# adamjorr/kbbq-py

Hardware: NVIDIA B200
Metric: bases/sec recalibrated (table build + apply) (higher is better)
Workload: dtype u8 in/out, u32->int64 counts, f64 model

## Files before the change

include/kbbq_b200.h:

```cpp
#ifndef KBBQ_B200_H
#define KBBQ_B200_H

#include <stddef.h>
#include <stdint.h>

#ifdef __cplusplus
extern "C" {
#endif

#define KBBQ_NQ 43
#define KBBQ_NDINUC 16

#define KBBQ_OK 0
#define KBBQ_E_ARG (-1)
#define KBBQ_E_CUDA (-2)
#define KBBQ_E_WORKSPACE (-3)
#define KBBQ_E_DATA (-4)
#define KBBQ_E_IO (-5)
#define KBBQ_E_FORMAT (-6)
#define KBBQ_E_RAGGED (-7)
#define KBBQ_E_NAME_FIELD (-8)
#define KBBQ_E_NAME_RG (-9)
#define KBBQ_E_NAME_MISMATCH (-10)
#define KBBQ_E_PEER (-11)
// ... 24 lines not shown
                   int64_t *rg_total_dev, int64_t *meanq_dev, void *stream);

int kbbq_delta_q(const int64_t *prior_q_dev, const int64_t *numerrs_dev,
                 const int64_t *numtotal_dev, int64_t n, int64_t *delta_dev, void *stream);

int kbbq_posterior_q_real(const double *prior_q_dev, const int64_t *numerrs_dev,
                          const int64_t *numtotal_dev, int64_t n, int64_t *posterior_dev, void *stream);

int kbbq_bam_workspace_bytes(int64_t N, int L, int R, size_t *bytes);
int kbbq_build_bam(const uint8_t *seq_dev, const uint8_t *qual_dev, const uint8_t *err_dev,
                   const uint8_t *skip_dev, const uint16_t *rg_dev, const uint8_t *flags_dev,
                   const uint16_t *aln_start_dev, const uint16_t *aln_end_dev, int64_t N, int L, int R,
                   int minscore, int64_t *pos_errs_dev, int64_t *pos_total_dev, int64_t *din_errs_dev,
                   int64_t *din_total_dev, void *workspace_dev, size_t workspace_bytes, int *status_dev,
                   void *stream);
int kbbq_apply_bam(const uint8_t *seq_dev, const uint8_t *qual_dev, const uint16_t *rg_dev,
                   const uint8_t *flags_dev, int64_t N, int L, int R, int minscore,
                   const int64_t *meanq_dev, const int64_t *rgdq_dev, const int64_t *qdq_dev,
                   const int64_t *posdq_dev, const int64_t *dindq_dev, int nq, int ndin1,
                   uint8_t *out_qual_dev, void *workspace_dev, size_t workspace_bytes, int *status_dev,
                   void *stream);

int kbbq_calibration_counts(const uint8_t *qual_dev, const uint8_t *err_dev, const uint8_t *seq_dev,
                            const uint8_t *corr_dev, const uint8_t *skip_dev, int64_t n,
                            int64_t *total_dev, int64_t *errs_dev, void *stream);

int kbbq_get_delta_qs(const int64_t *meanq_dev, const int64_t *rg_errs_dev,
                      const int64_t *rg_total_dev, const int64_t *q_errs_dev,
                      const int64_t *q_total_dev, const int64_t *pos_errs_dev,
                      const int64_t *pos_total_dev, const int64_t *din_errs_dev,
                      const int64_t *din_total_dev, int R, int nq, int ncyc, int ndin,
                      int64_t *rgdq_dev, int64_t *qdq_dev, int64_t *posdq_dev, int64_t *dindq_dev,
                      void *stream);

#define KBBQ_APPLY_BASES_CHECKED 0x10
int kbbq_apply(const uint8_t *seq_dev, const uint8_t *qual_dev, const uint16_t *rg_dev,
               const uint8_t *second_dev, int64_t N, int L, int R, int minscore,
               const int64_t *meanq_dev, const int64_t *rgdq_dev, const int64_t *qdq_dev,
               const int64_t *posdq_dev, const int64_t *dindq_dev, int nq, int ndin1,
               uint8_t *out_qual_dev, void *workspace_dev, size_t workspace_bytes, int *status_dev,
               int path, void *stream);

int64_t kbbq_segment_rows_bound(int64_t N, int R);
int64_t kbbq_segment_table_elems(int R);
int kbbq_segmented_supported(int L, int R, int minscore);
int kbbq_segment_plan(const uint16_t *rg_dev, const uint8_t *second_dev, int64_t N, int R, uint32_t *seg_dev,
                      uint32_t *dest_dev, int *status_dev, void *stream);
int kbbq_segment_rows(const uint8_t *src_dev, const uint32_t *dest_dev, int64_t N, int L, uint8_t *dst_segmented_dev,
                      void *stream);
int kbbq_segment_pad(const uint32_t *seg_dev, int R, int L, uint8_t *seq_dev, uint8_t *qual_dev, uint8_t *corr_dev,
                     void *stream);
int kbbq_unsegment_rows(const uint8_t *src_segmented_dev, const uint32_t *dest_dev, int64_t N, int L,
                        int64_t rows_bound, uint8_t *dst_dev, void *stream);
int kbbq_build_segmented(const uint8_t *seq_dev, const uint8_t *qual_dev, const uint8_t *corr_dev,
                         const uint32_t *seg_dev, int64_t rows_bound, int L, int R, int minscore,
                         int64_t *pos_errs_dev, int64_t *pos_total_dev, int64_t *din_errs_dev,
                         int64_t *din_total_dev, void *workspace_dev, size_t workspace_bytes, int *status_dev,
                         void *stream);
int kbbq_apply_segmented(const uint8_t *seq_dev, const uint8_t *qual_dev, const uint32_t *seg_dev, int64_t rows_bound,
                         int L, int R, int minscore, const int64_t *meanq_dev, const int64_t *rgdq_dev,
                         const int64_t *qdq_dev, const int64_t *posdq_dev, const int64_t *dindq_dev, int nq,
                         int ndin1, uint8_t *out_qual_dev, void *workspace_dev, size_t workspace_bytes,
                         int *status_dev, void *stream);
int kbbq_apply_segmented_flags(const uint8_t *seq_dev, const uint8_t *qual_dev, const uint32_t *seg_dev,
                               int64_t rows_bound, int L, int R, int minscore, const int64_t *meanq_dev,
                               const int64_t *rgdq_dev, const int64_t *qdq_dev, const int64_t *posdq_dev,
// ... 113 lines not shown
```

kbbq-py_b200/csrc/host_api.cu:

```cuda
#include <algorithm>
#include <atomic>
#include <chrono>
#include <condition_variable>
#include <memory>
#include <mutex>
#include <sched.h>
#include <stdlib.h>
#include <string.h>
#include <sys/mman.h>
#include <sys/stat.h>
#include <fcntl.h>
#include <thread>
#include <unistd.h>
#include <vector>

#include "common.cuh"

using namespace kbbq;

namespace {

#define KBBQ_TRY(x) do { int rc_ = (x); if (rc_) return rc_; } while (0)

constexpr int MAX_DEVICES = 16;
// ... 309 lines not shown
        uint8_t *sseq = keep ? r->seq : u.sseq, *squal = keep ? r->qual : u.squal;
        KBBQ_TRY(kbbq_segment_plan(p.d_rg, p.d_sec, n, R, seg, dest, S->d_status, S->s_comp));
        KBBQ_TRY(kbbq_segment_rows(p.d_seq, dest, n, L, sseq, S->s_comp));
        KBBQ_TRY(kbbq_segment_rows(p.d_qual, dest, n, L, squal, S->s_comp));
        KBBQ_TRY(kbbq_segment_rows(u.corr, dest, n, L, u.scorr, S->s_comp));
        KBBQ_TRY(kbbq_segment_pad(seg, R, L, sseq, squal, u.scorr, S->s_comp));
        KBBQ_TRY(kbbq_build_segmented(sseq, squal, u.scorr, seg, S->rowsC, L, R, S->minscore, pe, pt, de, dt, S->d_ws,
                                      S->ws_bytes, S->d_status, S->s_comp));
    } else {
        KBBQ_TRY(kbbq_build(p.d_seq, p.d_qual, u.corr, p.d_rg, p.d_sec, n, L, R, S->minscore, pe, pt, de, dt, S->d_ws, S->ws_bytes,
                            S->d_status, 0, S->s_comp));
    }
    KBBQ_CUDA(cudaEventRecord(u.consumed, S->s_comp));
    return KBBQ_OK;
}

int build_chunk_async(kbbq_session *S, const uint8_t *seq, const uint8_t *qual, const uint8_t *corr, const uint16_t *rg,
                      const uint8_t *second, int64_t n, bool keep) {
    if (n < 0 || n > S->C) return KBBQ_E_ARG;
    if (n == 0) return KBBQ_OK;
    if (!seq || !qual || !corr) return KBBQ_E_ARG;
    const int64_t k = S->built;
    if (keep && k >= (int64_t)S->res.size()) return KBBQ_E_ARG;
    S->built++;
    KBBQ_TRY(build_chunk_upload(S, k, seq, qual, rg, second, n, keep));
    return build_chunk_finish(S, k, seq, corr, rg != nullptr, second != nullptr, n, keep);
}

int model_async(kbbq_session *S) {
    const int L = S->L, R = S->R;
    const size_t npos = (size_t)R * NQ * 2 * L, ndin = (size_t)R * NQ * 16;
    int64_t *pe = S->summed ? S->d_sum : S->d_tab, *pt = pe + npos, *de = pt + npos, *dt = de + ndin;
    const ModelPtrs &mp = S->mp;
    KBBQ_TRY(kbbq_marginals(pe, pt, L, R, mp.q_errs, mp.q_total, mp.rg_errs, mp.rg_total, mp.meanq, S->s_comp));
    KBBQ_TRY(kbbq_get_delta_qs(mp.meanq, mp.rg_errs, mp.rg_total, mp.q_errs, mp.q_total, pe, pt, de, dt, R, NQ, 2 * L, 16,
                               mp.rgdq, mp.qdq, mp.posdq, mp.dindq, S->s_comp));
    return KBBQ_OK;
}

int apply_and_download(kbbq_session *S, const uint8_t *d_seq, const uint8_t *d_qual, const uint16_t *d_rg,
                       const uint8_t *d_sec, const uint32_t *seg, const uint32_t *dest, int64_t n, uint8_t *out_host) {
    const int L = S->L, R = S->R;
    OutSlot &o = S->down[S->applied++ & 1];
    const ModelPtrs &mp = S->mp;
    KBBQ_CUDA(cudaStreamWaitEvent(S->s_comp, o.drained, 0));
    if (S->segmode) {
        KBBQ_TRY(kbbq_apply_segmented(d_seq, d_qual, seg, S->rowsC, L, R, S->minscore, mp.meanq, mp.rgdq, mp.qdq, mp.posdq,
                                      mp.dindq, NQ, 17, o.out_seg, S->d_ws, S->ws_bytes, S->d_status, S->s_comp));
        KBBQ_TRY(kbbq_unsegment_rows(o.out_seg, dest, n, L, S->rowsC, o.out, S->s_comp));
    } else {
        KBBQ_TRY(kbbq_apply(d_seq, d_qual, d_rg, d_sec, n, L, R, S->minscore, mp.meanq, mp.rgdq, mp.qdq, mp.posdq, mp.dindq,
                            NQ, 17, o.out, S->d_ws, S->ws_bytes, S->d_status, 0, S->s_comp));
    }
    KBBQ_CUDA(cudaEventRecord(o.applied, S->s_comp));
    KBBQ_CUDA(cudaStreamWaitEvent(S->s_down, o.applied, 0));
    KBBQ_CUDA(cudaMemcpyAsync(out_host, o.out, (size_t)n * L, cudaMemcpyDeviceToHost, S->s_down));
    S->d2h_bytes += n * L;
    KBBQ_CUDA(cudaEventRecord(o.drained, S->s_down));
    return KBBQ_OK;
}

int apply_resident_async(kbbq_session *S, int64_t k, uint8_t *out_host) {
    if (k < 0 || k >= (int64_t)S->res.size() || !out_host) return KBBQ_E_ARG;
    const Resident &r = S->res[(size_t)k];
    if (r.n == 0) return KBBQ_OK;
    return apply_and_download(S, r.seq, r.qual, r.rg, r.sec, r.seg, r.dest, r.n, out_host);
}

int apply_chunk_async(kbbq_session *S, const uint8_t *seq, const uint8_t *qual, const uint16_t *rg, const uint8_t *second,
// ... 924 lines not shown
```

kbbq-py_b200/csrc/kbbq_b200.cu:

```cuda
#include <algorithm>
#include <mutex>
#include <stdlib.h>
#include <string.h>
#include <vector>

#include "apply.cuh"
#include "bam.cuh"
#include "build.cuh"
#include "calib.cuh"
#include "common.cuh"
#include "expand.cuh"
#include "model.cuh"
#include "prepare.cuh"
#include "segment.cuh"
#include "synth.cuh"

namespace kbbq {

std::atomic<long long> g_launches{0};
char g_last_cuda_error[256] = "";

static std::mutex g_const_mu;
static bool g_const_done[64];

// ... 105 lines not shown
};

template <class Generic>
static int plan_and_prepare(int narr, bool aligned, int64_t N, int L, int R, int minscore, const uint16_t *rg,
                            const uint8_t *second, void *workspace, size_t workspace_bytes, int *status, int path,
                            const unsigned int *seg_rows, cudaStream_t st, const Generic &generic, SmemPlan *p) {
    const bool segmode = seg_rows != nullptr;
    int device, max_smem;
    int rc = current_device_info(&device, &p->sms, &max_smem);
    if (rc) return rc;
    p->smem = path != 2 && aligned && plan_kernel(L, R, minscore, narr, max_smem, &p->g, &p->tc, &p->sl, segmode) &&
              (uint64_t)((N + p->g.G - 1) / p->g.G) < 0xFFFFFFFFull;
    if (!p->smem) {
        if (path == 1 || segmode) return KBBQ_E_ARG;
        return generic(0, N, p->sms * 8);
    }
    p->w = carve_workspace(workspace, N, L, R);
    if (!workspace || workspace_bytes < p->w.bytes) return KBBQ_E_WORKSPACE;
    p->N = N;
    if (segmode) {
        seg_prepare_kernel<<<1, 256, 0, st>>>(seg_rows, 2 * R, p->g.G, (unsigned long long)N, p->w.seg, p->w.uni, status);
        KBBQ_LAUNCHED();
        return KBBQ_OK;
    }
    const int64_t tail = (R == 1 && N > p->g.G) ? N % p->g.G : 0;
    if (tail) {
        p->N = N - tail;
        rc = generic(p->N, tail, 1);
        if (rc) return rc;
    }
    return run_prepare(rg, second, p->N, p->g.G, R, p->w, status, p->sms, p->sl.ngs, p->g.gbytes, p->sl.slot, st);
}

template <class Launch>
static int launch_bam_chunks(long long N, int L, const Launch &launch) {
    const unsigned int wmax = (unsigned int)((3 + L + 3) >> 2);
    const long long per = std::max<long long>(1, (long long)(0x7FFFFFFFu / wmax) / 256 * 256);
    for (long long r0 = 0; r0 < N; r0 += per) {
        const long long n = std::min<long long>(per, N - r0);
        launch((unsigned)((n * wmax + BAM_WARPS * 32 - 1) / (BAM_WARPS * 32)), r0, wmax);
        KBBQ_LAUNCHED();
    }
    return KBBQ_OK;
}

}

using namespace kbbq;

extern "C" {

int kbbq_abi_version(void) { return 1; }

const char *kbbq_strerror(int code) {
    switch (code) {
    case KBBQ_OK: return "ok";
    case KBBQ_E_ARG: return "bad argument";
    case KBBQ_E_CUDA: return "CUDA runtime error";
    case KBBQ_E_WORKSPACE: return "workspace too small";
    case KBBQ_E_DATA: return "input data error (see status flags)";
    case KBBQ_E_IO: return "FASTQ file could not be opened, read or written";
    case KBBQ_E_FORMAT: return "malformed FASTQ (4-line records expected)";
    case KBBQ_E_RAGGED: return "reads of unequal length";
    case KBBQ_E_NAME_FIELD: return "read name has no read-group field";
    case KBBQ_E_NAME_RG: return "read-group field does not start with RG";
    case KBBQ_E_NAME_MISMATCH: return "corrected read name does not start with the read name";
// ... 247 lines not shown
    const int grid = sms * 3;
    const long long chunk = (long long)grid * CAL_THREADS * CAL_MAX_ITERS * 32;
    auto kern = err ? (skip ? calibration_kernel<true, true> : calibration_kernel<true, false>)
                    : (skip ? calibration_kernel<false, true> : calibration_kernel<false, false>);
    KBBQ_CUDA(cudaFuncSetAttribute(kern, cudaFuncAttributeMaxDynamicSharedMemorySize, CAL_SMEM));
    for (long long o = 0; o < n; o += chunk) {
        CalibArgs c = a;
        c.qual += o; if (err) c.err += o; else { c.seq += o; c.corr += o; } if (skip) c.skip += o;
        c.n = std::min<long long>(chunk, n - o);
        kern<<<grid, CAL_THREADS, CAL_SMEM, st>>>(c);
        KBBQ_LAUNCHED();
    }
    return KBBQ_OK;
}

int kbbq_get_delta_qs(const int64_t *meanq, const int64_t *rg_errs, const int64_t *rg_total,
                      const int64_t *q_errs, const int64_t *q_total, const int64_t *pos_errs,
                      const int64_t *pos_total, const int64_t *din_errs, const int64_t *din_total, int R,
                      int nq, int ncyc, int ndin, int64_t *rgdq, int64_t *qdq, int64_t *posdq,
                      int64_t *dindq, void *stream) {
    if (R < 1 || nq < 1 || ncyc < 0 || ndin < 0) return KBBQ_E_ARG;
    if (!meanq || !rg_errs || !rg_total || !q_errs || !q_total || !rgdq || !qdq) return KBBQ_E_ARG;
    if ((ncyc && (!pos_errs || !pos_total || !posdq)) || !dindq || (ndin && (!din_errs || !din_total)))
        return KBBQ_E_ARG;
    int rc = upload_constants();
    if (rc) return rc;
    cudaStream_t st = (cudaStream_t)stream;
    DeltaArgs a = {(const long long *)meanq, (const long long *)rg_errs, (const long long *)rg_total,
                   (const long long *)q_errs, (const long long *)q_total, (const long long *)pos_errs,
                   (const long long *)pos_total, (const long long *)din_errs, (const long long *)din_total,
                   R, nq, ncyc, ndin, (long long *)rgdq, (long long *)qdq, (long long *)posdq, (long long *)dindq};
    delta_levels12_kernel<<<R, 64, 0, st>>>(a);
    KBBQ_LAUNCHED();
    const long long cells = (long long)R * nq * (ncyc + ndin + 1);
    delta_level3_kernel<<<(unsigned)((cells + 127) / 128), 128, 0, st>>>(a);
    KBBQ_LAUNCHED();
    return KBBQ_OK;
}

static int apply_impl(const uint8_t *seq, const uint8_t *qual, const uint16_t *rg, const uint8_t *second, int64_t N,
                      int L, int R, int minscore, const int64_t *meanq, const int64_t *rgdq, const int64_t *qdq,
                      const int64_t *posdq, const int64_t *dindq, int nq, int ndin1, uint8_t *out_qual,
                      void *workspace, size_t workspace_bytes, int *status, int path, void *stream,
                      const unsigned int *seg_rows) {
    const bool segmode = seg_rows != nullptr;
    const bool validate = !(path & KBBQ_APPLY_BASES_CHECKED);
    path &= ~KBBQ_APPLY_BASES_CHECKED;
    if (N < 0 || L < 1 || R < 1 || R > 65535 || minscore < 0 || minscore >= NQ) return KBBQ_E_ARG;
    if (nq < 1 || nq > NQ || ndin1 < 16 || ndin1 > 64) return KBBQ_E_ARG;
    if (!meanq || !rgdq || !qdq || !posdq || !dindq || !status) return KBBQ_E_ARG;
    if (N == 0) return KBBQ_OK;
    if (!seq || !qual || !out_qual) return KBBQ_E_ARG;
    cudaStream_t st = (cudaStream_t)stream;
    Workspace w = carve_workspace(workspace, N, L, R);
    if (!workspace || workspace_bytes < w.bytes) return KBBQ_E_WORKSPACE;

    const long long fold_cells = (long long)R * NQ * (2 * L + 16);
    fold_kernel<<<(unsigned)((fold_cells + 255) / 256), 256, 0, st>>>(
        (const long long *)meanq, (const long long *)rgdq, (const long long *)qdq, (const long long *)posdq,
        (const long long *)dindq, R, nq, 2 * L, ndin1, w.fold_cyc, w.fold_din);
    KBBQ_LAUNCHED();

    auto generic = [&](int64_t r0, int64_t n, int grid) {
        ApplyGenericArgs a = {seq + r0 * L, qual + r0 * L, rg ? rg + r0 : nullptr, second ? second + r0 : nullptr,
                              out_qual + r0 * L, n, L, R, minscore, nq, w.fold_cyc, w.fold_din, status, validate};
        apply_generic_kernel<<<grid, 256, 0, st>>>(a);
        KBBQ_LAUNCHED();
        return KBBQ_OK;
// ... 146 lines not shown
```

kbbq-py_b200/csrc/model.cuh:

```cuda
#pragma once
#include "common.cuh"

namespace kbbq {

__constant__ double c_lnp[NQ];
__constant__ double c_ln1mp[NQ];
__constant__ double c_prior[NQ];
__constant__ double c_p[NQ];
__constant__ double c_bound_hi[NQ];
__constant__ double c_bound_lo[NQ];

struct dd { double hi, lo; };
__device__ __forceinline__ dd two_sum(double a, double b) {
    double s = __dadd_rn(a, b), bb = __dsub_rn(s, a);
    double e = __dadd_rn(__dsub_rn(a, __dsub_rn(s, bb)), __dsub_rn(b, bb));
    return {s, e};
}
__device__ __forceinline__ dd two_prod(double a, double b) {
    double p = __dmul_rn(a, b);
    return {p, __fma_rn(a, b, -p)};
}
__device__ __forceinline__ dd dd_add(dd a, dd b) {
    dd s = two_sum(a.hi, b.hi);
    double lo = __dadd_rn(s.lo, __dadd_rn(a.lo, b.lo));
    return two_sum(s.hi, lo);
}
__device__ __forceinline__ dd dd_div_d(dd a, double b) {
    double q1 = __ddiv_rn(a.hi, b);
    dd p = two_prod(q1, b);
    double r = __dadd_rn(__dsub_rn(__dsub_rn(a.hi, p.hi), p.lo), a.lo);
    double q2 = __ddiv_rn(r, b);
    return two_sum(q1, q2);
}
__device__ __forceinline__ bool dd_le(dd a, double bh, double bl) {
    return a.hi < bh || (a.hi == bh && a.lo <= bl);
}

__global__ void marginals_q_kernel(const long long *pos_errs, const long long *pos_total, int L2,
                                   long long *q_errs, long long *q_total) {
    const int q = blockIdx.x, rg = blockIdx.y;
    const size_t base = ((size_t)rg * NQ + q) * L2;
    long long e = 0, t = 0;
    for (int c = threadIdx.x; c < L2; c += blockDim.x) { e += pos_errs[base + c]; t += pos_total[base + c]; }
    __shared__ long long se[32], st[32];
    for (int o = 16; o; o >>= 1) { e += __shfl_down_sync(0xFFFFFFFFu, e, o); t += __shfl_down_sync(0xFFFFFFFFu, t, o); }
    if ((threadIdx.x & 31) == 0) { se[threadIdx.x >> 5] = e; st[threadIdx.x >> 5] = t; }
    __syncthreads();
    if (threadIdx.x == 0) {
        e = 0; t = 0;
        for (int w = 0; w < (blockDim.x + 31) / 32; ++w) { e += se[w]; t += st[w]; }
        q_errs[rg * NQ + q] = e;
        q_total[rg * NQ + q] = t;
    }
}

__global__ void marginals_rg_kernel(const long long *q_errs, const long long *q_total, int R,
                                    long long *rg_errs, long long *rg_total, long long *meanq) {
    const int rg = blockIdx.x;
    __shared__ long long s_e[NQ], s_t[NQ];
    if (threadIdx.x < NQ) {
        s_e[threadIdx.x] = q_errs[rg * NQ + threadIdx.x];
        s_t[threadIdx.x] = q_total[rg * NQ + threadIdx.x];
    }
    __syncthreads();
    if (threadIdx.x != 0) return;
    long long e = 0, t = 0;
    dd acc = {0.0, 0.0};
    for (int q = 0; q < NQ; ++q) {
        const long long tq = s_t[q];
        e += s_e[q];
        t += tq;
        if (tq) acc = dd_add(acc, two_prod((double)tq, c_p[q]));
    }
    rg_errs[rg] = e;
    rg_total[rg] = t;
    long long mq = 0;
    if (t > 0) {
        if (acc.hi == 0.0) mq = NQ - 1;
        else {
            const dd p = dd_div_d(acc, (double)t);
            for (int m = 1; m < NQ; ++m) mq += dd_le(p, c_bound_hi[m], c_bound_lo[m]) ? 1 : 0;
        }
    }
    meanq[rg] = mq;
}

__device__ __forceinline__ dd round_to_x87(dd s) {
    if (s.lo == 0.0 || isinf(s.hi) || isnan(s.hi)) return s;
    int e;
    frexp(s.hi, &e);
    int eh = e - 1;
    if (fabs(s.hi) == ldexp(1.0, eh) && ((s.hi > 0.0) != (s.lo > 0.0))) eh -= 1;
    const int qe = eh - 63;
    const double lo_r = ldexp(rint(ldexp(s.lo, -qe)), qe);
    const double h = __dadd_rn(s.hi, lo_r);
    return {h, __dadd_rn(__dsub_rn(s.hi, h), lo_r)};
}

template <typename PRIOR>
__device__ __forceinline__ int posterior_q_cell(PRIOR prior, long long errs, long long tot) {
    const double k = (double)(errs + 1), mm = (double)((tot + 2) - (errs + 1));
    int best = 0;
    double bh = 0.0, bl = 0.0;
    bool have = false;
    for (int c = 0; c < NQ; ++c) {
        int d = (int)((PRIOR)c - prior);
        d = d < 0 ? -d : d;
        const double pr = d < NQ ? c_prior[d] : -KBBQ_INF;
        const double a = __dmul_rn(k, c_lnp[c]);
        const double b = (mm == 0.0) ? 0.0 : __dmul_rn(mm, c_ln1mp[c]);
        const double ll = __dadd_rn(a, b);
        double h, l;
        if (isinf(pr) || isinf(ll)) { h = -KBBQ_INF; l = 0.0; }
        else { dd s = round_to_x87(two_sum(pr, ll)); h = s.hi; l = s.lo; }
        if (!have || h > bh || (h == bh && l > bl)) { best = c; bh = h; bl = l; have = true; }
    }
    return best;
}
__device__ __forceinline__ int delta_q_cell(int prior, long long errs, long long tot) {
    return posterior_q_cell<int>(prior, errs, tot) - prior;
}

__global__ void delta_q_kernel(const long long *prior, const long long *errs, const long long *tot,
                               long long n, long long *out) {
    long long i = (long long)blockIdx.x * blockDim.x + threadIdx.x;
    if (i < n) out[i] = delta_q_cell((int)prior[i], errs[i], tot[i]);
}

__global__ void posterior_q_real_kernel(const double *prior, const long long *errs, const long long *tot,
                                        long long n, long long *out) {
    long long i = (long long)blockIdx.x * blockDim.x + threadIdx.x;
    if (i < n) out[i] = posterior_q_cell<double>(prior[i], errs[i], tot[i]);
}

struct DeltaArgs {
    const long long *meanq, *rg_errs, *rg_total, *q_errs, *q_total, *pos_errs, *pos_total, *din_errs, *din_total;
    int R, nq, ncyc, ndin;
    long long *rgdq, *qdq, *posdq, *dindq;
};

__global__ void delta_levels12_kernel(DeltaArgs a) {
    const int rg = blockIdx.x;
    __shared__ int s_prior1;
    if (threadIdx.x == 0) {
        const int mq = (int)a.meanq[rg];
        const int d = delta_q_cell(mq, a.rg_errs[rg], a.rg_total[rg]);
        a.rgdq[rg] = d;
        s_prior1 = mq + d;
    }
    __syncthreads();
    for (int q = threadIdx.x; q < a.nq; q += blockDim.x)
        a.qdq[rg * a.nq + q] = delta_q_cell(s_prior1, a.q_errs[rg * a.nq + q], a.q_total[rg * a.nq + q]);
}

__global__ void delta_level3_kernel(DeltaArgs a) {
    const long long ncell_pos = (long long)a.R * a.nq * a.ncyc;
    const long long ncell_din = (long long)a.R * a.nq * (a.ndin + 1);
    long long i = (long long)blockIdx.x * blockDim.x + threadIdx.x;
    if (i < ncell_pos) {
        const long long gq = i / a.ncyc;
        const int rg = (int)(gq / a.nq);
        const int prior2 = (int)(a.meanq[rg] + a.rgdq[rg] + a.qdq[gq]);
        a.posdq[i] = delta_q_cell(prior2, a.pos_errs[i], a.pos_total[i]);
    } else if (i < ncell_pos + ncell_din) {
        i -= ncell_pos;
        const long long gq = i / (a.ndin + 1);
        const int d = (int)(i - gq * (a.ndin + 1));
        if (d == a.ndin) { a.dindq[i] = 0; return; }
        const int rg = (int)(gq / a.nq);
        const int prior2 = (int)(a.meanq[rg] + a.rgdq[rg] + a.qdq[gq]);
        a.dindq[i] = delta_q_cell(prior2, a.din_errs[gq * a.ndin + d], a.din_total[gq * a.ndin + d]);
    }
}

__global__ void fold_kernel(const long long *meanq, const long long *rgdq, const long long *qdq,
                            const long long *posdq, const long long *dindq, int R, int nq, int L2,
                            int ndin1, short *fold_cyc, short *fold_din) {
    const long long ncyc = (long long)R * NQ * L2, ndin = (long long)R * NQ * 16;
    long long i = (long long)blockIdx.x * blockDim.x + threadIdx.x;
    if (i < ncyc) {
        const long long gq = i / L2;
        const int c2 = (int)(i - gq * L2);
        const int rg = (int)(gq / NQ), q = (int)(gq - (long long)rg * NQ);
        long long v = 0;
        if (q < nq)
            v = meanq[rg] + rgdq[rg] + qdq[rg * nq + q] + posdq[((size_t)rg * nq + q) * L2 + c2] +
                dindq[((size_t)rg * nq + q) * ndin1 + ndin1 - 1];
        fold_cyc[i] = (short)v;
    } else if (i < ncyc + ndin) {
        i -= ncyc;
        const long long gq = i >> 4;
        const int n = (int)(i & 15);
        const int rg = (int)(gq / NQ), q = (int)(gq - (long long)rg * NQ);
        long long v = 0;
        if (q < nq) {
            const size_t row = ((size_t)rg * nq + q) * ndin1;
            v = dindq[row + nat_to_ref(n >> 2) * 4 + nat_to_ref(n & 3)] - dindq[row + ndin1 - 1];
        }
        fold_din[i] = (short)v;
    }
}

}
```

kbbq-py_b200/kbbq/_native.py:

```python
import ctypes as C
import os

import numpy as np

HERE = os.path.dirname(os.path.abspath(__file__))
LIB_PATH = os.path.join(HERE, "libkbbq_b200.so")

NQ = 43
FLAG_QUAL_RANGE, FLAG_BAD_BASE, FLAG_RG_RANGE, FLAG_SEGMENTS = 1, 2, 4, 8
APPLY_BASES_CHECKED = 0x10
E_DATA = -4
E_UNSUPPORTED = -12

_lib = None

_vp, _i, _i64, _sz = C.c_void_p, C.c_int, C.c_int64, C.c_size_t
SIGNATURES = {
    "kbbq_abi_version": (_i, []),
    "kbbq_strerror": (C.c_char_p, [_i]),
    "kbbq_last_cuda_error": (C.c_char_p, []),
    "kbbq_pos_table_elems": (_i64, [_i, _i]),
    "kbbq_din_table_elems": (_i64, [_i]),
    "kbbq_workspace_bytes": (_i, [_i64, _i, _i, C.POINTER(_sz)]),
    "kbbq_build": (_i, [_vp] * 5 + [_i64, _i, _i, _i] + [_vp] * 4 + [_vp, _sz, _vp, _i, _vp]),
    "kbbq_marginals": (_i, [_vp, _vp, _i, _i] + [_vp] * 5 + [_vp]),
    "kbbq_delta_q": (_i, [_vp, _vp, _vp, _i64, _vp, _vp]),
    "kbbq_get_delta_qs": (_i, [_vp] * 9 + [_i, _i, _i, _i] + [_vp] * 4 + [_vp]),
    "kbbq_apply": (_i, [_vp] * 4 + [_i64, _i, _i, _i] + [_vp] * 5 + [_i, _i, _vp, _vp, _sz, _vp, _i, _vp]),
    "kbbq_recalibrate_host": (_i, [_vp] * 5 + [_i64, _i, _i, _i] + [_vp] * 3 + [C.POINTER(_i), _i]),
    "kbbq_recalibrate_host_multi": (_i, [_vp] * 5 + [_i64, _i, _i, _i] + [_vp] * 3 + [C.POINTER(_i), C.POINTER(_i), _i]),
    "kbbq_recalibrate_fastq": (_i, [C.c_char_p, C.c_char_p, _i, _i, _i, _i, _i, C.POINTER(_i64), C.POINTER(_i), C.POINTER(_i)]),
    "kbbq_host_release": (_i, [_i]),
    "kbbq_session_create": (_i, [_i, _i, _i, _i, _i64, _i64, _i, C.POINTER(_vp)]),
    "kbbq_session_destroy": (None, [_vp]),
    "kbbq_session_chunk_reads": (_i64, [_vp]),
    "kbbq_session_reset": (_i, [_vp]),
    "kbbq_session_build_chunk": (_i, [_vp] * 6 + [_i64, _i]),
    "kbbq_session_build_range": (_i, [_vp] * 6 + [_i64]),
    "kbbq_session_tables": (_i, [_vp, _vp]),
    "kbbq_session_set_tables": (_i, [_vp, _vp]),
    "kbbq_session_tables_dev": (_i, [_vp, C.POINTER(_vp), C.POINTER(_i64), C.POINTER(_vp)]),
    "kbbq_session_model": (_i, [_vp, _vp]),
    "kbbq_session_apply_resident": (_i, [_vp, _i64, _vp]),
    "kbbq_session_apply_chunk": (_i, [_vp] * 5 + [_i64, _vp]),
    "kbbq_session_flush": (_i, [_vp]),
    "kbbq_session_sync": (_i, [_vp, C.POINTER(_i)]),
    "kbbq_session_traffic": (_i, [_vp, C.POINTER(_i64), C.POINTER(_i64)]),
    "kbbq_build_host": (_i, [_vp] * 5 + [_i64, _i, _i, _i] + [_vp] * 4 + [C.POINTER(_i), _i]),
    "kbbq_apply_host": (_i, [_vp] * 4 + [_i64, _i, _i, _i] + [_vp] * 5 + [_i, _i, _vp, C.POINTER(_i), _i]),
    "kbbq_get_delta_qs_host": (_i, [_vp] * 9 + [_i, _i, _i, _i] + [_vp] * 4 + [_i]),
    "kbbq_delta_q_host": (_i, [_vp, _vp, _vp, _i64, _vp, _i]),
    "kbbq_posterior_q_real": (_i, [_vp, _vp, _vp, _i64, _vp, _vp]),
    "kbbq_posterior_q_real_host": (_i, [_vp, _vp, _vp, _i64, _vp, _i]),
    "kbbq_calibration_counts": (_i, [_vp] * 5 + [_i64, _vp, _vp, _vp]),
    "kbbq_calibration_counts_host": (_i, [_vp] * 5 + [_i64, _vp, _vp, _i]),
    "kbbq_bam_workspace_bytes": (_i, [_i64, _i, _i, C.POINTER(_sz)]),
    "kbbq_build_bam": (_i, [_vp] * 8 + [_i64, _i, _i, _i] + [_vp] * 4 + [_vp, _sz, _vp, _vp]),
    "kbbq_apply_bam": (_i, [_vp] * 4 + [_i64, _i, _i, _i] + [_vp] * 5 + [_i, _i, _vp, _vp, _sz, _vp, _vp]),
    "kbbq_build_bam_host": (_i, [_vp] * 8 + [_i64, _i, _i, _i] + [_vp] * 4 + [_vp, _i]),
    "kbbq_apply_bam_host": (_i, [_vp] * 4 + [_i64, _i, _i, _i] + [_vp] * 5 + [_i, _i, _vp, _vp, _i]),
# ... 376 lines not shown
```

kbbq-py_b200/kbbq/device.py:

```python
import ctypes as C
import weakref

import torch

from . import _native
from . import parallel

NQ = _native.NQ


def _p(t):
    return None if t is None else C.c_void_p(t.data_ptr())


def _on_device(fn):
    import functools

    @functools.wraps(fn)
    def wrapper(self, *args, **kwargs):
        with torch.cuda.device(self.device):
            return fn(self, *args, **kwargs)
    return wrapper


# ... 106 lines not shown
        _native.check(self.lib.kbbq_segment_pad(_p(seg), R, L, _p(outs[0]), _p(outs[1]), _p(outs[2]), st))
        return SegmentedBatch(outs[0], outs[1], outs[2], seg, dest, N, rows)

    @_on_device
    def build_segmented(self, sb):
        self._ensure_workspace(sb.rows_bound)
        rc = self.lib.kbbq_build_segmented(_p(sb.seq), _p(sb.qual), _p(sb.corr), _p(sb.seg), sb.rows_bound, self.L, self.R,
                                           self.minscore, _p(self.pos_errs), _p(self.pos_total), _p(self.din_errs),
                                           _p(self.din_total), _p(self.workspace), self.ws_bytes, _p(self.status),
                                           self._stream())
        _native.check(rc)
        self._remember_built(sb.seq)

    @_on_device
    def apply_segmented(self, sb, out_seg):
        self._ensure_workspace(sb.rows_bound)
        flags = _native.APPLY_BASES_CHECKED if self._bases_checked(sb.seq) else 0
        rc = self.lib.kbbq_apply_segmented_flags(_p(sb.seq), _p(sb.qual), _p(sb.seg), sb.rows_bound, self.L, self.R,
                                                 self.minscore, _p(self.meanq), _p(self.rgdq), _p(self.qdq),
                                                 _p(self.posdq), _p(self.dindq), NQ, 17, _p(out_seg), _p(self.workspace),
                                                 self.ws_bytes, _p(self.status), flags, self._stream())
        _native.check(rc)

    @_on_device
    def unsegment(self, sb, out_seg, out):
        _native.check(self.lib.kbbq_unsegment_rows(_p(out_seg), _p(sb.dest), sb.N, self.L, sb.rows_bound, _p(out),
                                                   self._stream()))

    def allreduce(self):
        parallel.allreduce_tables(self.tables, self.pg)

    @_on_device
    def model(self):
        L, R = self.L, self.R
        _native.check(self.lib.kbbq_marginals(_p(self.pos_errs), _p(self.pos_total), L, R, _p(self.q_errs),
                                              _p(self.q_total), _p(self.rg_errs), _p(self.rg_total),
                                              _p(self.meanq), self._stream()))
        _native.check(self.lib.kbbq_get_delta_qs(_p(self.meanq), _p(self.rg_errs), _p(self.rg_total),
                                                 _p(self.q_errs), _p(self.q_total), _p(self.pos_errs),
                                                 _p(self.pos_total), _p(self.din_errs), _p(self.din_total),
                                                 R, NQ, 2 * L, 16, _p(self.rgdq), _p(self.qdq), _p(self.posdq),
                                                 _p(self.dindq), self._stream()))

    @_on_device
    def apply(self, seq, qual, out, rg=None, second=None, path=0):
        N = seq.numel() // self.L
        self._ensure_workspace(N)
        if self._bases_checked(seq):
            path |= _native.APPLY_BASES_CHECKED
        rc = self.lib.kbbq_apply(_p(seq), _p(qual), _p(rg), _p(second), N, self.L, self.R, self.minscore,
                                 _p(self.meanq), _p(self.rgdq), _p(self.qdq), _p(self.posdq), _p(self.dindq),
                                 NQ, 17, _p(out), _p(self.workspace), self.ws_bytes, _p(self.status), path,
                                 self._stream())
        _native.check(rc)

    @_on_device
    def build_bam(self, seq, qual, err, skip=None, rg=None, flags=None, aln_start=None, aln_end=None, fast=True):
        N = seq.numel() // self.L
        ws = self._bam_workspace(N) if fast else None
        rc = self.lib.kbbq_build_bam(_p(seq), _p(qual), _p(err), _p(skip), _p(rg), _p(flags), _p(aln_start),
                                     _p(aln_end), N, self.L, self.R, self.minscore, _p(self.pos_errs),
                                     _p(self.pos_total), _p(self.din_errs), _p(self.din_total), _p(ws),
                                     0 if ws is None else ws.numel(), _p(self.status), self._stream())
        _native.check(rc)

    @_on_device
    def _bam_workspace(self, n_reads):
        if n_reads > getattr(self, "bam_ws_reads", -1):
            nbytes = C.c_size_t(0)
            _native.check(self.lib.kbbq_bam_workspace_bytes(n_reads, self.L, self.R, C.byref(nbytes)))
            self.bam_ws = torch.empty(max(nbytes.value, 256), dtype=torch.uint8, device=self.device)
            self.bam_ws_reads = n_reads
        return self.bam_ws

    @_on_device
# ... 53 lines not shown
```

Before: 871.3 billion.

## Fuse marginals and delta-q levels into one per-read-group model kernel

Replaces the separate marginals and delta-q launches with one model_kernel. Each read-group block reduces the position tables, computes the mean quality and the level-1/2 priors in shared memory, then handles its share of the level-3 cells. The posterior argmax over the 43 quality values is split across 1, 4 or 16 lanes and combined with warp shuffles, with the lane count picked from the SM count and cell count. This removes several kernel launches and round-trips through global memory for small model tables, but every y-block repeats the level-1/2 work, and the tie-breaking in the lane-parallel argmax has to match the original serial order.

```diff
diff --git a/include/kbbq_b200.h b/include/kbbq_b200.h
--- a/include/kbbq_b200.h
+++ b/include/kbbq_b200.h
@@ -80,6 +80,11 @@
                       const int64_t *din_total_dev, int R, int nq, int ncyc, int ndin,
                       int64_t *rgdq_dev, int64_t *qdq_dev, int64_t *posdq_dev, int64_t *dindq_dev,
                       void *stream);
+
+int kbbq_model(const int64_t *pos_errs_dev, const int64_t *pos_total_dev, const int64_t *din_errs_dev,
+               const int64_t *din_total_dev, int L, int R, int64_t *q_errs_dev, int64_t *q_total_dev,
+               int64_t *rg_errs_dev, int64_t *rg_total_dev, int64_t *meanq_dev, int64_t *rgdq_dev,
+               int64_t *qdq_dev, int64_t *posdq_dev, int64_t *dindq_dev, void *stream);
 
 #define KBBQ_APPLY_BASES_CHECKED 0x10
 int kbbq_apply(const uint8_t *seq_dev, const uint8_t *qual_dev, const uint16_t *rg_dev,
diff --git a/kbbq-py_b200/csrc/host_api.cu b/kbbq-py_b200/csrc/host_api.cu
--- a/kbbq-py_b200/csrc/host_api.cu
+++ b/kbbq-py_b200/csrc/host_api.cu
@@ -365,9 +365,8 @@
     const size_t npos = (size_t)R * NQ * 2 * L, ndin = (size_t)R * NQ * 16;
     int64_t *pe = S->summed ? S->d_sum : S->d_tab, *pt = pe + npos, *de = pt + npos, *dt = de + ndin;
     const ModelPtrs &mp = S->mp;
-    KBBQ_TRY(kbbq_marginals(pe, pt, L, R, mp.q_errs, mp.q_total, mp.rg_errs, mp.rg_total, mp.meanq, S->s_comp));
-    KBBQ_TRY(kbbq_get_delta_qs(mp.meanq, mp.rg_errs, mp.rg_total, mp.q_errs, mp.q_total, pe, pt, de, dt, R, NQ, 2 * L, 16,
-                               mp.rgdq, mp.qdq, mp.posdq, mp.dindq, S->s_comp));
+    KBBQ_TRY(kbbq_model(pe, pt, de, dt, L, R, mp.q_errs, mp.q_total, mp.rg_errs, mp.rg_total, mp.meanq, mp.rgdq,
+                        mp.qdq, mp.posdq, mp.dindq, S->s_comp));
     return KBBQ_OK;
 }
 
diff --git a/kbbq-py_b200/csrc/kbbq_b200.cu b/kbbq-py_b200/csrc/kbbq_b200.cu
--- a/kbbq-py_b200/csrc/kbbq_b200.cu
+++ b/kbbq-py_b200/csrc/kbbq_b200.cu
@@ -161,6 +161,15 @@
     return run_prepare(rg, second, p->N, p->g.G, R, p->w, status, p->sms, p->sl.ngs, p->g.gbytes, p->sl.slot, st);
 }
 
+static dim3 model_plan(long long cells, int R, int sms, int *lanes) {
+    const long long threads = (long long)sms * 2048;
+    *lanes = cells * R * 16 <= threads ? 16 : cells * R * 4 <= threads ? 4 : 1;
+    const long long bps = *lanes == 1 ? 6 : 1;
+    const long long rounds = (cells * *lanes + MODEL_THREADS - 1) / MODEL_THREADS;
+    const long long per_rg = std::max(1ll, std::min(rounds, (bps * sms + R - 1) / R));
+    return dim3((unsigned)R, (unsigned)per_rg);
+}
+
 template <class Launch>
 static int launch_bam_chunks(long long N, int L, const Launch &launch) {
     const unsigned int wmax = (unsigned int)((3 + L + 3) >> 2);
@@ -474,8 +483,41 @@
                    R, nq, ncyc, ndin, (long long *)rgdq, (long long *)qdq, (long long *)posdq, (long long *)dindq};
     delta_levels12_kernel<<<R, 64, 0, st>>>(a);
     KBBQ_LAUNCHED();
-    const long long cells = (long long)R * nq * (ncyc + ndin + 1);
-    delta_level3_kernel<<<(unsigned)((cells + 127) / 128), 128, 0, st>>>(a);
+    int device, sms, max_smem;
+    rc = current_device_info(&device, &sms, &max_smem);
+    if (rc) return rc;
+    int lanes;
+    const dim3 grid = model_plan((long long)nq * (ncyc + ndin + 1), R, sms, &lanes);
+    if (lanes == 16) delta_level3_kernel<16><<<grid, MODEL_THREADS, 0, st>>>(a);
+    else if (lanes == 4) delta_level3_kernel<4><<<grid, MODEL_THREADS, 0, st>>>(a);
+    else delta_level3_kernel<1><<<grid, MODEL_THREADS, 0, st>>>(a);
+    KBBQ_LAUNCHED();
+    return KBBQ_OK;
+}
+
+int kbbq_model(const int64_t *pos_errs, const int64_t *pos_total, const int64_t *din_errs, const int64_t *din_total,
+               int L, int R, int64_t *q_errs, int64_t *q_total, int64_t *rg_errs, int64_t *rg_total, int64_t *meanq,
+               int64_t *rgdq, int64_t *qdq, int64_t *posdq, int64_t *dindq, void *stream) {
+    if (L < 1 || R < 1 || R > 65535 || !pos_errs || !pos_total || !din_errs || !din_total || !q_errs || !q_total ||
+        !rg_errs || !rg_total || !meanq || !rgdq || !qdq || !posdq || !dindq)
+        return KBBQ_E_ARG;
+    int rc = upload_constants();
+    if (rc) return rc;
+    int device, sms, max_smem;
+    rc = current_device_info(&device, &sms, &max_smem);
+    if (rc) return rc;
+    ModelArgs m;
+    m.d = {nullptr, nullptr, nullptr, nullptr, nullptr, (const long long *)pos_errs, (const long long *)pos_total,
+           (const long long *)din_errs, (const long long *)din_total, R, NQ, 2 * L, 16, (long long *)rgdq,
+           (long long *)qdq, (long long *)posdq, (long long *)dindq};
+    m.q_errs = (long long *)q_errs; m.q_total = (long long *)q_total;
+    m.rg_errs = (long long *)rg_errs; m.rg_total = (long long *)rg_total; m.meanq = (long long *)meanq;
+    int lanes;
+    const dim3 grid = model_plan((long long)NQ * (2 * L + 17), R, sms, &lanes);
+    cudaStream_t st = (cudaStream_t)stream;
+    if (lanes == 16) model_kernel<16><<<grid, MODEL_THREADS, 0, st>>>(m);
+    else if (lanes == 4) model_kernel<4><<<grid, MODEL_THREADS, 0, st>>>(m);
+    else model_kernel<1><<<grid, MODEL_THREADS, 0, st>>>(m);
     KBBQ_LAUNCHED();
     return KBBQ_OK;
 }
diff --git a/kbbq-py_b200/csrc/model.cuh b/kbbq-py_b200/csrc/model.cuh
--- a/kbbq-py_b200/csrc/model.cuh
+++ b/kbbq-py_b200/csrc/model.cuh
@@ -54,26 +54,21 @@
     }
 }
 
-__global__ void marginals_rg_kernel(const long long *q_errs, const long long *q_total, int R,
-                                    long long *rg_errs, long long *rg_total, long long *meanq) {
-    const int rg = blockIdx.x;
-    __shared__ long long s_e[NQ], s_t[NQ];
-    if (threadIdx.x < NQ) {
-        s_e[threadIdx.x] = q_errs[rg * NQ + threadIdx.x];
-        s_t[threadIdx.x] = q_total[rg * NQ + threadIdx.x];
-    }
-    __syncthreads();
-    if (threadIdx.x != 0) return;
+__device__ __forceinline__ void q_products(const long long *s_t, dd *s_prod) {
+    if (threadIdx.x < NQ) s_prod[threadIdx.x] = two_prod((double)s_t[threadIdx.x], c_p[threadIdx.x]);
+}
+__device__ __forceinline__ void rg_marginals(const long long *s_e, const long long *s_t, const dd *s_prod,
+                                             long long &rg_errs, long long &rg_total, long long &meanq) {
     long long e = 0, t = 0;
     dd acc = {0.0, 0.0};
     for (int q = 0; q < NQ; ++q) {
         const long long tq = s_t[q];
         e += s_e[q];
         t += tq;
-        if (tq) acc = dd_add(acc, two_prod((double)tq, c_p[q]));
-    }
-    rg_errs[rg] = e;
-    rg_total[rg] = t;
+        if (tq) acc = dd_add(acc, s_prod[q]);
+    }
+    rg_errs = e;
+    rg_total = t;
     long long mq = 0;
     if (t > 0) {
         if (acc.hi == 0.0) mq = NQ - 1;
@@ -82,7 +77,22 @@
             for (int m = 1; m < NQ; ++m) mq += dd_le(p, c_bound_hi[m], c_bound_lo[m]) ? 1 : 0;
         }
     }
-    meanq[rg] = mq;
+    meanq = mq;
+}
+
+__global__ void marginals_rg_kernel(const long long *q_errs, const long long *q_total, int R,
+                                    long long *rg_errs, long long *rg_total, long long *meanq) {
+    const int rg = blockIdx.x;
+    __shared__ long long s_e[NQ], s_t[NQ];
+    __shared__ dd s_prod[NQ];
+    if (threadIdx.x < NQ) {
+        s_e[threadIdx.x] = q_errs[rg * NQ + threadIdx.x];
+        s_t[threadIdx.x] = q_total[rg * NQ + threadIdx.x];
+    }
+    __syncthreads();
+    q_products(s_t, s_prod);
+    __syncthreads();
+    if (threadIdx.x == 0) rg_marginals(s_e, s_t, s_prod, rg_errs[rg], rg_total[rg], meanq[rg]);
 }
 
 __device__ __forceinline__ dd round_to_x87(dd s) {
@@ -98,24 +108,42 @@
 }
 
 template <typename PRIOR>
+__device__ __forceinline__ dd posterior_value(PRIOR prior, double k, double mm, int c) {
+    int d = (int)((PRIOR)c - prior);
+    d = d < 0 ? -d : d;
+    const double pr = d < NQ ? c_prior[d] : -KBBQ_INF;
+    const double a = __dmul_rn(k, c_lnp[c]);
+    const double b = (mm == 0.0) ? 0.0 : __dmul_rn(mm, c_ln1mp[c]);
+    const double ll = __dadd_rn(a, b);
+    if (isinf(pr) || isinf(ll)) return {-KBBQ_INF, 0.0};
+    return round_to_x87(two_sum(pr, ll));
+}
+__device__ __forceinline__ bool posterior_ahead(dd v, int c, dd w, int cw) {
+    if (v.hi != w.hi) return v.hi > w.hi;
+    if (v.lo != w.lo) return v.lo > w.lo;
+    return c < cw;
+}
+
+template <typename PRIOR, int LANES>
+__device__ __forceinline__ int posterior_q_lanes(PRIOR prior, long long errs, long long tot, int sub) {
+    const double k = (double)(errs + 1), mm = (double)((tot + 2) - (errs + 1));
+    int best = sub;
+    dd bv = posterior_value<PRIOR>(prior, k, mm, sub);
+    for (int c = sub + LANES; c < NQ; c += LANES) {
+        const dd v = posterior_value<PRIOR>(prior, k, mm, c);
+        if (v.hi > bv.hi || (v.hi == bv.hi && v.lo > bv.lo)) { best = c; bv = v; }
+    }
+#pragma unroll
+    for (int o = LANES / 2; o; o >>= 1) {
+        const dd w = {__shfl_xor_sync(0xFFFFFFFFu, bv.hi, o), __shfl_xor_sync(0xFFFFFFFFu, bv.lo, o)};
+        const int cw = __shfl_xor_sync(0xFFFFFFFFu, best, o);
+        if (posterior_ahead(w, cw, bv, best)) { best = cw; bv = w; }
+    }
+    return best;
+}
+template <typename PRIOR>
 __device__ __forceinline__ int posterior_q_cell(PRIOR prior, long long errs, long long tot) {
-    const double k = (double)(errs + 1), mm = (double)((tot + 2) - (errs + 1));
-    int best = 0;
-    double bh = 0.0, bl = 0.0;
-    bool have = false;
-    for (int c = 0; c < NQ; ++c) {
-        int d = (int)((PRIOR)c - prior);
-        d = d < 0 ? -d : d;
-        const double pr = d < NQ ? c_prior[d] : -KBBQ_INF;
-        const double a = __dmul_rn(k, c_lnp[c]);
-        const double b = (mm == 0.0) ? 0.0 : __dmul_rn(mm, c_ln1mp[c]);
-        const double ll = __dadd_rn(a, b);
-        double h, l;
-        if (isinf(pr) || isinf(ll)) { h = -KBBQ_INF; l = 0.0; }
-        else { dd s = round_to_x87(two_sum(pr, ll)); h = s.hi; l = s.lo; }
-        if (!have || h > bh || (h == bh && l > bl)) { best = c; bh = h; bl = l; have = true; }
-    }
-    return best;
+    return posterior_q_lanes<PRIOR, 1>(prior, errs, tot, 0);
 }
 __device__ __forceinline__ int delta_q_cell(int prior, long long errs, long long tot) {
     return posterior_q_cell<int>(prior, errs, tot) - prior;
@@ -153,24 +181,125 @@
         a.qdq[rg * a.nq + q] = delta_q_cell(s_prior1, a.q_errs[rg * a.nq + q], a.q_total[rg * a.nq + q]);
 }
 
-__global__ void delta_level3_kernel(DeltaArgs a) {
-    const long long ncell_pos = (long long)a.R * a.nq * a.ncyc;
-    const long long ncell_din = (long long)a.R * a.nq * (a.ndin + 1);
-    long long i = (long long)blockIdx.x * blockDim.x + threadIdx.x;
-    if (i < ncell_pos) {
-        const long long gq = i / a.ncyc;
-        const int rg = (int)(gq / a.nq);
-        const int prior2 = (int)(a.meanq[rg] + a.rgdq[rg] + a.qdq[gq]);
-        a.posdq[i] = delta_q_cell(prior2, a.pos_errs[i], a.pos_total[i]);
-    } else if (i < ncell_pos + ncell_din) {
-        i -= ncell_pos;
-        const long long gq = i / (a.ndin + 1);
-        const int d = (int)(i - gq * (a.ndin + 1));
-        if (d == a.ndin) { a.dindq[i] = 0; return; }
-        const int rg = (int)(gq / a.nq);
-        const int prior2 = (int)(a.meanq[rg] + a.rgdq[rg] + a.qdq[gq]);
-        a.dindq[i] = delta_q_cell(prior2, a.din_errs[gq * a.ndin + d], a.din_total[gq * a.ndin + d]);
-    }
+constexpr int MODEL_THREADS = 512;
+
+template <int LANES, class Prior2>
+__device__ __forceinline__ void level3_cells(const DeltaArgs &a, int rg, long long lo, long long hi, const Prior2 &prior2) {
+    const long long npos = (long long)a.nq * a.ncyc;
+    const int sub = threadIdx.x % LANES;
+    for (long long j0 = lo; j0 < hi; j0 += MODEL_THREADS / LANES) {
+        const long long j = j0 + threadIdx.x / LANES;
+        long long errs = 0, tot = 0, *out = nullptr;
+        int prior = 0;
+        if (j < hi) {
+            if (j < npos) {
+                const size_t i = (size_t)rg * npos + j;
+                prior = prior2(j / a.ncyc);
+                errs = a.pos_errs[i];
+                tot = a.pos_total[i];
+                out = a.posdq + i;
+            } else {
+                const long long jd = j - npos, q = jd / (a.ndin + 1);
+                const int d = (int)(jd - q * (a.ndin + 1));
+                long long *o = a.dindq + (size_t)rg * a.nq * (a.ndin + 1) + jd;
+                if (d == a.ndin) {
+                    if (sub == 0) *o = 0;
+                } else {
+                    const size_t i = ((size_t)rg * a.nq + q) * a.ndin + d;
+                    prior = prior2(q);
+                    errs = a.din_errs[i];
+                    tot = a.din_total[i];
+                    out = o;
+                }
+            }
+        }
+        if (LANES == 1 && !out) continue;
+        const int p = posterior_q_lanes<int, LANES>(prior, errs, tot, sub);
+        if (out && sub == 0) *out = p - prior;
+    }
+}
+
+template <int LANES>
+__global__ void __launch_bounds__(MODEL_THREADS) delta_level3_kernel(DeltaArgs a) {
+    const int rg = blockIdx.x;
+    const long long n = (long long)a.nq * (a.ncyc + a.ndin + 1);
+    const long long *qdq = a.qdq + (size_t)rg * a.nq;
+    const long long mq = a.meanq[rg], rgdq = a.rgdq[rg];
+    level3_cells<LANES>(a, rg, n * blockIdx.y / gridDim.y, n * (blockIdx.y + 1) / gridDim.y,
+                        [&](long long q) { return (int)(mq + rgdq + qdq[q]); });
+}
+
+struct ModelArgs {
+    DeltaArgs d;
+    long long *q_errs, *q_total, *rg_errs, *rg_total, *meanq;
+};
+
+template <int LANES>
+__global__ void __launch_bounds__(MODEL_THREADS, 3) model_kernel(const __grid_constant__ ModelArgs m) {
+    const DeltaArgs &a = m.d;
+    const int rg = blockIdx.x, warp = threadIdx.x >> 5, lane = threadIdx.x & 31;
+    __shared__ long long s_e[NQ], s_t[NQ], s_rg[3];
+    __shared__ dd s_prod[NQ];
+    __shared__ int s_prior1, s_prior2[NQ];
+    constexpr int WARPS = MODEL_THREADS / 32, ROWS = (NQ + WARPS - 1) / WARPS;
+    {
+        long long e[ROWS] = {}, t[ROWS] = {};
+#pragma unroll 2
+        for (int c = lane; c < a.ncyc; c += 32) {
+#pragma unroll
+            for (int k = 0; k < ROWS; ++k) {
+                const int q = warp + k * WARPS;
+                if (q < NQ) {
+                    const size_t i = ((size_t)rg * NQ + q) * a.ncyc + c;
+                    e[k] += a.pos_errs[i];
+                    t[k] += a.pos_total[i];
+                }
+            }
+        }
+#pragma unroll
+        for (int k = 0; k < ROWS; ++k) {
+            for (int o = 16; o; o >>= 1) {
+                e[k] += __shfl_down_sync(0xFFFFFFFFu, e[k], o);
+                t[k] += __shfl_down_sync(0xFFFFFFFFu, t[k], o);
+            }
+            const int q = warp + k * WARPS;
+            if (lane == 0 && q < NQ) { s_e[q] = e[k]; s_t[q] = t[k]; }
+        }
+    }
+    __syncthreads();
+    q_products(s_t, s_prod);
+    __syncthreads();
+    if (threadIdx.x == 0) rg_marginals(s_e, s_t, s_prod, s_rg[0], s_rg[1], s_rg[2]);
+    __syncthreads();
+    if (warp == 0) {
+        const int p = posterior_q_lanes<int, 16>((int)s_rg[2], s_rg[0], s_rg[1], lane & 15);
+        if (lane == 0) s_prior1 = p;
+    }
+    __syncthreads();
+    const int prior1 = s_prior1;
+    static_assert(NQ * 8 <= MODEL_THREADS, "level 2 in one pass");
+    if (warp < (NQ * 8 + 31) / 32) {
+        const int q = threadIdx.x / 8, qc = q < NQ ? q : 0;
+        const int p = posterior_q_lanes<int, 8>(prior1, s_e[qc], s_t[qc], threadIdx.x & 7);
+        if (q < NQ && (threadIdx.x & 7) == 0) s_prior2[q] = p;
+    }
+    __syncthreads();
+    if (blockIdx.y == 0) {
+        for (int q = threadIdx.x; q < NQ; q += MODEL_THREADS) {
+            m.q_errs[rg * NQ + q] = s_e[q];
+            m.q_total[rg * NQ + q] = s_t[q];
+            a.qdq[rg * NQ + q] = s_prior2[q] - prior1;
+        }
+        if (threadIdx.x == 0) {
+            m.rg_errs[rg] = s_rg[0];
+            m.rg_total[rg] = s_rg[1];
+            m.meanq[rg] = s_rg[2];
+            a.rgdq[rg] = prior1 - s_rg[2];
+        }
+    }
+    const long long n = (long long)NQ * (a.ncyc + a.ndin + 1);
+    level3_cells<LANES>(a, rg, n * blockIdx.y / gridDim.y, n * (blockIdx.y + 1) / gridDim.y,
+                        [&](long long q) { return s_prior2[q]; });
 }
 
 __global__ void fold_kernel(const long long *meanq, const long long *rgdq, const long long *qdq,
diff --git a/kbbq-py_b200/kbbq/_native.py b/kbbq-py_b200/kbbq/_native.py
--- a/kbbq-py_b200/kbbq/_native.py
+++ b/kbbq-py_b200/kbbq/_native.py
@@ -26,6 +26,7 @@
     "kbbq_marginals": (_i, [_vp, _vp, _i, _i] + [_vp] * 5 + [_vp]),
     "kbbq_delta_q": (_i, [_vp, _vp, _vp, _i64, _vp, _vp]),
     "kbbq_get_delta_qs": (_i, [_vp] * 9 + [_i, _i, _i, _i] + [_vp] * 4 + [_vp]),
+    "kbbq_model": (_i, [_vp] * 4 + [_i, _i] + [_vp] * 9 + [_vp]),
     "kbbq_apply": (_i, [_vp] * 4 + [_i64, _i, _i, _i] + [_vp] * 5 + [_i, _i, _vp, _vp, _sz, _vp, _i, _vp]),
     "kbbq_recalibrate_host": (_i, [_vp] * 5 + [_i64, _i, _i, _i] + [_vp] * 3 + [C.POINTER(_i), _i]),
     "kbbq_recalibrate_host_multi": (_i, [_vp] * 5 + [_i64, _i, _i, _i] + [_vp] * 3 + [C.POINTER(_i), C.POINTER(_i), _i]),
diff --git a/kbbq-py_b200/kbbq/device.py b/kbbq-py_b200/kbbq/device.py
--- a/kbbq-py_b200/kbbq/device.py
+++ b/kbbq-py_b200/kbbq/device.py
@@ -162,15 +162,10 @@
 
     @_on_device
     def model(self):
-        L, R = self.L, self.R
-        _native.check(self.lib.kbbq_marginals(_p(self.pos_errs), _p(self.pos_total), L, R, _p(self.q_errs),
-                                              _p(self.q_total), _p(self.rg_errs), _p(self.rg_total),
-                                              _p(self.meanq), self._stream()))
-        _native.check(self.lib.kbbq_get_delta_qs(_p(self.meanq), _p(self.rg_errs), _p(self.rg_total),
-                                                 _p(self.q_errs), _p(self.q_total), _p(self.pos_errs),
-                                                 _p(self.pos_total), _p(self.din_errs), _p(self.din_total),
-                                                 R, NQ, 2 * L, 16, _p(self.rgdq), _p(self.qdq), _p(self.posdq),
-                                                 _p(self.dindq), self._stream()))
+        _native.check(self.lib.kbbq_model(_p(self.pos_errs), _p(self.pos_total), _p(self.din_errs),
+                                          _p(self.din_total), self.L, self.R, _p(self.q_errs), _p(self.q_total),
+                                          _p(self.rg_errs), _p(self.rg_total), _p(self.meanq), _p(self.rgdq),
+                                          _p(self.qdq), _p(self.posdq), _p(self.dindq), self._stream()))
 
     @_on_device
     def apply(self, seq, qual, out, rg=None, second=None, path=0):
```

Result: faster. 890.0 billion (median of 6 runs) (+2.1%).
